# xuzhougeng/minimap2_rs

Hardware: AMD Instinct MI355X
Metric: aligned Gbases/sec (PAF out), 10k×10kb ONT reads vs hg38, 1/2/4/8 GPUs (higher is better)
Workload: dtype int32

## Files before the change

include/mm2g.h:

```cpp
#ifndef MM2G_H
#define MM2G_H
#include <stdint.h>

#ifdef __cplusplus
extern "C" {
#endif

#define MM2G_OK 0
#define MM2G_E_ARG -1
#define MM2G_E_IO -2
#define MM2G_E_HIP -3
#define MM2G_E_NOMEM -4
#define MM2G_E_STATE -5
#define MM2G_E_UNSUP -6

typedef struct mm2g_index mm2g_index;
typedef struct mm2g_ctx mm2g_ctx;

int mm2g_version(void);
const char* mm2g_last_error(void);
int mm2g_device_count(void);

int mm2g_index_build_fasta(const char* path, int w, int k, int b, int flag, int n_threads, mm2g_index** out);
int mm2g_index_build_seqs(uint32_t n_seq, const char* const* names, const uint8_t* const* seqs, const uint64_t* lens,
// ... 146 lines not shown
    MM2G_KNOB_SKETCH_VIEW = 27,
    MM2G_KNOB_PRUNE_RESCUE = 29,
    MM2G_KNOB_VIEW_READS = 30,
    MM2G_KNOB_SEG_SPARSE = 31,
    MM2G_KNOB_SPEC_BATCH = 32,
    MM2G_KNOB_DV_PAR = 33,
    MM2G_KNOB_SEED_FUSE = 36,
    MM2G_KNOB_SKETCH_X32 = 37,
    MM2G_KNOB_BIG_WND = 38,
    MM2G_KNOB_CANDS_LONGW = 39,
    MM2G_KNOB_SEED_FUSE_BIG = 40,
    MM2G_KNOB_READ_TINY = 41,
    MM2G_KNOB_BIG_TINY = 42,
    MM2G_KNOB_SPEC_EVAL = 43,
    MM2G_KNOB_SMALL_REG = 44,
    MM2G_KNOB_COUNT = 45
};
int mm2g_ctx_set_knob(mm2g_ctx* ctx, int knob, int64_t value);
int64_t mm2g_ctx_get_knob(const mm2g_ctx* ctx, int knob);
enum {
    MM2G_IKNOB_IXCHUNK = 1,
    MM2G_IKNOB_IXPROF = 2,
    MM2G_IKNOB_LOAD_THREADS = 3,
    MM2G_IKNOB_GPU_STRICT = 4,
    MM2G_IKNOB_FORCE_FALLBACK = 5,
    MM2G_IKNOB_IXSORTV = 6,
    MM2G_IKNOB_COUNT = 7
};
int mm2g_set_index_knob(int knob, int64_t value);

int mm2g_prof_enable(mm2g_ctx* ctx, int on);
// ... 10 lines not shown
```

minimap2_rs_amd/_lib.py:

```python
from __future__ import annotations

import ctypes as C
import os

HERE = os.path.dirname(os.path.abspath(__file__))
BUILD_DIR = os.path.join(HERE, "build")
LIB_PATH = os.environ.get("MM2G_LIB") or os.path.join(BUILD_DIR, "libmm2g.so")
CLI_PATH = os.path.join(BUILD_DIR, "mm2rs")

MM2G_R_MAPPED = 1
MM2G_R_RESCUED = 2
MM2G_R_DV_FOUND = 4
MM2G_R_PANIC = 8
MM2G_R_EMPTY = 16


class MapOpts(C.Structure):
    _fields_ = [("w", C.c_int32), ("k", C.c_int32), ("max_gap", C.c_int32), ("bw", C.c_int32), ("bw_long", C.c_int32),
                ("min_cnt", C.c_int32), ("min_chain_score", C.c_int32), ("mask_level", C.c_float),
                ("pri_ratio", C.c_float), ("best_n", C.c_int32)]


class ReadResult(C.Structure):
    _fields_ = [("flags", C.c_int32), ("n_anchors", C.c_int32), ("score", C.c_int32), ("cm", C.c_int32),
# ... 19 lines not shown

class ChainResult(C.Structure):
    _fields_ = [("flags", C.c_int32), ("n_anchors", C.c_int32), ("score", C.c_int32), ("cm", C.c_int32), ("qs", C.c_int32),
                ("qe", C.c_int32), ("ts", C.c_int32), ("te", C.c_int32), ("rid", C.c_int32), ("rev", C.c_int32)]


class ChainLine(C.Structure):
    _fields_ = [("qs", C.c_int32), ("qe", C.c_int32), ("ts", C.c_int32), ("te", C.c_int32), ("rid", C.c_int32),
                ("rev", C.c_int32), ("cm", C.c_int32), ("primary", C.c_int32), ("dv", C.c_float), ("s1", C.c_int32),
                ("s2", C.c_int32)]


KNOBS = {"sort_small": 1, "seg_small": 2, "seg_chunk": 3, "giant_min": 4, "giant_min0": 5, "giant_lcap": 6, "giant_gmax": 7,
         "giant_gblocks": 8, "filter": 9, "lazy": 10, "prune": 11, "giant": 12, "sketch_prof": 13, "sort_prof": 14,
         "lseg_prof": 15, "midhist_bins": 16, "sync_each": 17, "host_threads": 18, "ws_min": 19,
         "sort_lds_kb": 20, "stop_at": 21, "spec_rounds": 22, "med_pairs": 23, "med_pairs_rescue": 24, "ws_fail": 25, "sketch_view": 27, "prune_rescue": 29, "view_reads": 30, "seg_sparse": 31, "spec_batch": 32, "dv_par": 33, "seed_fuse": 36, "sketch_x32": 37, "big_wnd": 38, "cands_longw": 39, "seed_fuse_big": 40, "read_tiny": 41, "big_tiny": 42, "spec_eval": 43, "small_reg": 44}
INDEX_KNOBS = {"ixchunk": 1, "ixprof": 2, "load_threads": 3, "gpu_strict": 4, "force_fallback": 5, "ixsortv": 6}
INDEX_ORIGINS = {1: "host build", 2: "gpu build", 3: "gpu build fell back to the host build", 4: ".mmi load"}

_VP = C.c_void_p
_P64 = C.POINTER(C.c_uint64)
_PI32 = C.POINTER(C.c_int32)

SIGNATURES = {
    "mm2g_version": (C.c_int, []),
    "mm2g_last_error": (C.c_char_p, []),
    "mm2g_device_count": (C.c_int, []),
    "mm2g_index_build_fasta": (C.c_int, [C.c_char_p, C.c_int, C.c_int, C.c_int, C.c_int, C.c_int, C.POINTER(_VP)]),
    "mm2g_index_build_seqs": (C.c_int, [C.c_uint32, C.POINTER(C.c_char_p), C.POINTER(C.c_void_p), _P64,
                                        C.c_int, C.c_int, C.c_int, C.c_int, C.c_int, C.POINTER(_VP)]),
    "mm2g_index_build_fasta_gpu": (C.c_int, [C.c_char_p, C.c_int, C.c_int, C.c_int, C.c_int, C.c_int, C.c_int, C.POINTER(_VP)]),
# ... 78 lines not shown
```

minimap2_rs_amd/csrc/mm2g_host.hip:

```cpp
#include <hip/hip_runtime.h>

#include <algorithm>
#include <cmath>
#include <cstdarg>
#include <cstdio>
#include <cstring>
#include <map>
#include <memory>
#include <mutex>
#include <string>
#include <atomic>
#include <thread>
#include <vector>

#include "../../include/mm2g.h"
#include "mm2g_index.h"
#include "mm2g_internal.h"
#include "mm2g_multi.h"
#include "mm2g_reads.h"

using namespace mm2g;

static thread_local std::string g_err;
static int set_err(int code, const char* fmt, ...) {
// ... 78 lines not shown
    case MM2G_KNOB_SKETCH_VIEW: return 2560;
    case MM2G_KNOB_PRUNE_RESCUE: return 1;
    case MM2G_KNOB_VIEW_READS: return 2048;
    case MM2G_KNOB_SEG_SPARSE: return 1;
    case MM2G_KNOB_SPEC_BATCH: return 4;
    case MM2G_KNOB_DV_PAR: return 1;
    case MM2G_KNOB_SEED_FUSE: return 1;
    case MM2G_KNOB_SEED_FUSE_BIG: return 1;
    case MM2G_KNOB_READ_TINY: return 16;
    case MM2G_KNOB_BIG_TINY: return 16;
    case MM2G_KNOB_SPEC_EVAL: return 1;
    case MM2G_KNOB_SMALL_REG: return 1;
    case MM2G_KNOB_SKETCH_X32: return 1;
    case MM2G_KNOB_BIG_WND: return 126;
    case MM2G_KNOB_CANDS_LONGW: return 1024;
    case MM2G_KNOB_HOST_THREADS: return (int64_t)std::max(1u, std::min(8u, std::thread::hardware_concurrency()));
    default: return 0;
    }
}

struct mm2g_ctx {
    int device = 0;
    hipStream_t stream = nullptr;
    int64_t knob[MM2G_KNOB_COUNT] = {};
    const HostIndex* hidx = nullptr;
    struct DevIndex { DevBuf tab, ix_pos, goff; uint32_t cells = 0; };
    std::shared_ptr<DevIndex> dix;
    uint32_t log2cap = 0;
    int32_t mid_occ = 10;
    bool have_index = false;
// ... 953 lines not shown
}

static int enqueue_sort(mm2g_ctx* c, const mm2g_map_opts* o, MapBatch& B) {
    const uint32_t n = B.n;
    const int64_t* K = c->knob;
    SeedArgs sa = seed_args(c, o, B);
    sa.keys = B.keys; sa.cap_keys = c->keys.cap / 8;
    sa.order = B.rorder;
    sa.fuse_mmax = B.fuse_mmax; sa.small_max = B.sort_small_max; sa.fuse_big = B.fuse_big;
    {
        ProfScope ps(c, "seed_write");
        LCHK(launch_seed_write(sa, grid_for(n), c->stream));
    }
    uint32_t* rlist;
    ENSURE(c->cnt2, uint32_t, n, B.cnt2);
    ENSURE(c->rlist, uint32_t, n + 2, rlist);
    ENSURE(c->smax, uint64_t, n, B.smax);
    SortArgs so{};
    so.n = n; so.a_off = B.a_off; so.keys = B.keys; so.tmp = B.ktmp;
    so.qb = B.kl.qb; so.rb = B.kl.rb; so.n_seq = B.kl.n_seq;
    so.cap_keys = c->keys.cap / 8;
    so.goff = (const uint32_t*)c->dix->goff.p;
    so.cells = B.filt ? c->dix->cells : 0u;
    so.cnt2 = B.cnt2; so.smax = B.smax;
    so.small_max = B.sort_small_max;
    so.seg_small = (uint32_t)std::max<int64_t>(1, std::min<int64_t>(K[MM2G_KNOB_SEG_SMALL], SEG_THREAD));
    so.abort = B.st32;
    so.meta = (uint32_t*)c->fbuf.p;
    so.rlist = rlist; so.rcount = rlist + n; so.rwork = rlist + n + 1;
    so.order = B.rorder;
    so.lds_words = (uint32_t)(std::max<int64_t>(0, K[MM2G_KNOB_SORT_LDS_KB]) * 256);
    so.fuse_mmax = B.fuse_mmax;
    so.fuse_big = B.fuse_big; so.a_part = B.a_part;
    so.read_tiny = (uint32_t)std::max<int64_t>(1, std::min<int64_t>(K[MM2G_KNOB_READ_TINY], 1024));
    so.big_tiny = (uint32_t)std::max<int64_t>(1, std::min<int64_t>(K[MM2G_KNOB_BIG_TINY], 2048));
    so.small_reg = K[MM2G_KNOB_SMALL_REG] ? 1u : 0u;
    so.big_wnd = (uint32_t)std::max<int64_t>(0, K[MM2G_KNOB_BIG_WND]);
    so.rd_off = c->d_rd_off; so.mz_base = B.mz_base; so.mz_cnt = B.mz_cnt; so.mz_y = B.mz_y;
    so.mz_n = B.mz_n; so.mz_poff = B.mz_poff; so.ix_pos = (const uint64_t*)c->dix->ix_pos.p; so.kl = B.kl; so.span = o->k;
    so.cap_pos = c->dix->ix_pos.cap / 8;
    uint64_t* sprof = nullptr;
    if (K[MM2G_KNOB_SORT_PROF]) { HIPCHK(hipMalloc(&sprof, (size_t)n * 192)); HIPCHK(hipMemsetAsync(sprof, 0, (size_t)n * 192, c->stream)); so.prof = sprof; }
    if (K[MM2G_KNOB_STOP_AT] == 1) return 0;
    {
        ProfScope ps(c, "sort_small");
// ... 71 lines not shown
    }
    if (n == 0) {
        HIPCHK(hipMemcpyAsync(c->h_stat, B.st, STAT_WORDS * 8, hipMemcpyDeviceToHost, c->stream));
        HIPCHK(hipEventRecord(c->ev_done, c->stream));
        c->mapped = true;
        return 0;
    }
    if (int e = run_sketch(c, o->w, o->k, c->sk1, (int32_t*)B.st32, B.out, B.st)) return e;
    B.mcap = c->sk1.cap;
    B.mz_base = (const uint64_t*)c->sk1.base.p; B.mz_cnt = (const uint32_t*)c->sk1.cnt.p;
    B.mz_x = (const uint64_t*)c->sk1.x.p; B.mz_y = (const uint32_t*)c->sk1.y.p;
    if (int e = enqueue_filter(c, o, B)) return e;
    if (int e = enqueue_seed_count(c, o, B)) return e;
    B.filt = !full && !stop_after_sort && K[MM2G_KNOB_FILTER] && std::max(mdx0, mdx1) <= (1 << CELL_SHIFT);
    B.sort_small_max = (uint32_t)std::min<int64_t>(K[MM2G_KNOB_SORT_SMALL], 4096);
    if (B.filt && K[MM2G_KNOB_SEED_FUSE]) {
        SortArgs t{};
        t.cells = c->dix->cells;
        t.lds_words = (uint32_t)(std::max<int64_t>(0, K[MM2G_KNOB_SORT_LDS_KB]) * 256);
        const uint32_t LW = sort_read_lds_words(t), nw = (t.cells + 31) / 32;
        if (LW > 2 * nw + 64 + 2048) B.fuse_mmax = std::min<uint32_t>((LW - 2 * nw - 64 - 2048) / 4, 0xffffu);
    }
    B.fuse_big = (B.filt && K[MM2G_KNOB_SEED_FUSE_BIG]) ? 1u : 0u;
    c->filt_last = B.filt; c->small_last = B.sort_small_max;
    if (int e = enqueue_sort(c, o, B)) return e;
    const int64_t stop_at = K[MM2G_KNOB_STOP_AT];
    const bool chain = !stop_after_sort && stop_at != 1 && stop_at != 2;
    if (chain) {
        ChainJob J;
        J.n = n; J.rd_off = c->d_rd_off; J.a_off = B.a_off; J.a_cnt = B.a_cnt;
        J.keys = B.keys; J.ktmp = B.ktmp; J.cnt2 = B.cnt2; J.smax = B.smax;
        J.out = B.out; J.abort = B.st32; J.stat = B.st;
        J.P0.max_dist_x = mdx0; J.P0.max_dist_y = std::max(o->max_gap, o->bw); J.P0.bw = o->bw; J.P0.max_iter = 5000; J.P0.max_skip = 25;
        J.P0.span = o->k; J.P0.rescue_size = 1000; J.P0.rescue_ratio_f = 1.0f - 0.1f; J.P0.pass = 0; J.P0.lut_n = o->bw + 1;
        J.P0.multi = multi ? 1 : 0;
        J.gap = 0.01f * 0.8f * (float)o->k;
        J.npass = stop_at == 3 ? 1 : 2;
        J.mdx1 = mdx1; J.mdy1 = std::max(o->max_gap, o->bw_long); J.bw_long = o->bw_long;
// ... 713 lines not shown
```

minimap2_rs_amd/csrc/mm2g_internal.h:

```cpp
#pragma once
#include <stdint.h>

namespace mm2g {

constexpr uint64_t U64MAX = ~0ULL;
constexpr int WAVE = 64;
constexpr int CHAIN_TINY = 8;
constexpr int CHAIN_MED = 128;

struct KeyLayout {
    uint32_t qb, rb, gb;
    uint32_t n_seq;
};

struct ReadOut {
    int32_t flags;
    int32_t n_anchors;
    int32_t score;
    int32_t cm;
    int32_t qs, qe, ts, te;
    int32_t group;
    int32_t best_i;
    int32_t n_match;
    int32_t dv_st, dv_en;
// ... 122 lines not shown
    uint64_t cap_keys = 0;
    const uint32_t* goff = nullptr;
    uint32_t cells = 0;
    uint32_t* cnt2 = nullptr;
    uint64_t* smax = nullptr;
    uint32_t small_max = 0;
    uint64_t* prof = nullptr;
    uint32_t lds_words = 0;
    uint32_t seg_small = 0;
    uint32_t* meta = nullptr;
    const uint32_t* abort = nullptr;
    uint32_t* rlist = nullptr;
    uint32_t* rcount = nullptr;
    const uint32_t* order = nullptr;
    uint32_t* rwork = nullptr;
    uint32_t big_wnd = 1u << 30;
    uint32_t fuse_mmax = 0;
    const uint64_t* rd_off = nullptr; const uint64_t* mz_base = nullptr; const uint32_t* mz_cnt = nullptr;
    const uint32_t* mz_y = nullptr; const uint32_t* mz_n = nullptr; const uint32_t* mz_poff = nullptr;
    const uint64_t* ix_pos = nullptr; KeyLayout kl{}; int span = 0; uint64_t cap_pos = 0;
    uint32_t fuse_big = 0;
    const uint32_t* a_part = nullptr;
    uint32_t read_tiny = 16, big_tiny = 16;
    uint32_t small_reg = 1;
};
struct ChainArgs {
    uint32_t n = 0;
    const uint64_t* rd_off = nullptr;
    const uint64_t* a_off = nullptr;
    const uint64_t* keys = nullptr;
// ... 111 lines not shown
```

minimap2_rs_amd/csrc/mm2g_kernels.hip:

```cpp
#include <hip/hip_runtime.h>
#include <stdint.h>
#include <limits.h>
#include <algorithm>
#include <type_traits>
#include "mm2g_internal.h"

using namespace mm2g;

#define DEVI __device__ __forceinline__

#ifdef MM2G_CHECKED
__device__ unsigned long long g_chk[4];
DEVI uint64_t ck_idx(uint64_t i, uint64_t cap, int line) {
    if (i < cap) return i;
    if (atomicCAS(&g_chk[0], 0ULL, (unsigned long long)line) == 0ULL) { g_chk[1] = i; g_chk[2] = cap; }
    return 0;
}
#define CK(i, cap) ck_idx((uint64_t)(i), (uint64_t)(cap), __LINE__)
#define TRACE(tr, slot, v) do { if (tr) __hip_atomic_store(&(tr)[slot], (uint32_t)(v), __ATOMIC_RELAXED, __HIP_MEMORY_SCOPE_SYSTEM); } while (0)
#else
#define TRACE(tr, slot, v) do {} while (0)
#define CK(i, cap) (i)
#endif

// ... 7 lines not shown
DEVI void wave_lds_sync() {
    __builtin_amdgcn_fence(__ATOMIC_RELEASE, "wavefront");
    __builtin_amdgcn_wave_barrier();
    __builtin_amdgcn_fence(__ATOMIC_ACQUIRE, "wavefront");
}
DEVI void vm_drain() { asm volatile("s_waitcnt vmcnt(0)" ::: "memory"); }

DEVI int32_t rdl(int32_t v, int l) { return __builtin_amdgcn_readlane(v, l); }
DEVI uint32_t rdlu(uint32_t v, int l) { return (uint32_t)__builtin_amdgcn_readlane((int)v, l); }
DEVI uint64_t rdl64(uint64_t v, int l) {
    uint32_t lo = (uint32_t)__builtin_amdgcn_readlane((int)(uint32_t)v, l);
    uint32_t hi = (uint32_t)__builtin_amdgcn_readlane((int)(uint32_t)(v >> 32), l);
    return ((uint64_t)hi << 32) | lo;
}
DEVI int32_t uni(int32_t v) { return __builtin_amdgcn_readfirstlane(v); }

DEVI int32_t shr1(int32_t v, int32_t in0) {
    const int32_t t = __shfl_up(v, 1, 64);
    return lane_id() == 0 ? in0 : t;
}

template <typename T, typename F>
DEVI T wave_incl_scan(T v, F op) {
    const int l = lane_id();
#pragma unroll
    for (int d = 1; d < 64; d <<= 1) {
        T o = __shfl_up(v, d, 64);
        if (l >= d) v = op(o, v);
    }
    return v;
}
// ... 857 lines not shown
#pragma unroll
                for (int r = 0; r < KPT; ++r) {
                    const uint64_t y = s[(t ^ m) * KPT + r];
                    x[r] = (lowt == up) ? (x[r] < y ? x[r] : y) : (x[r] > y ? x[r] : y);
                }
            }
        }
    }
    __syncthreads();
#pragma unroll
    for (int r = 0; r < KPT; ++r) s[t * KPT + r] = x[r];
    __syncthreads();
}

__global__ __launch_bounds__(256) void k_sort_small(SortArgs a) {
    if (blockIdx.x == 0 && threadIdx.x == 0) { *a.rcount = 0; if (a.rwork) *a.rwork = 0; }
    if (a.abort && (*a.abort & BS_ANCHORS)) return;
    __shared__ uint64_t s[SORT_SMALL];
    const uint32_t r = blockIdx.x;
    if (r >= a.n) return;
    const uint64_t base = a.a_off[r];
    const uint32_t A = (uint32_t)(a.a_off[r + 1] - base);
    if (A > a.small_max) return;
    if (threadIdx.x == 0) { a.cnt2[r] = A; a.smax[r] = 0; }
    if (A == 1 && threadIdx.x == 0) a.tmp[CK(base, a.cap_keys)] = a.keys[CK(base, a.cap_keys)];
    if (A <= 1) return;
    uint32_t np = 1; while (np < A) np <<= 1;
    uint64_t* K = a.keys;
    for (uint32_t i = threadIdx.x; i < np; i += blockDim.x) s[i] = i < A ? K[CK(base + i, a.cap_keys)] : U64MAX;
    __syncthreads();
    if (np >= 512 && a.small_reg) {
// ... 328 lines not shown
#undef NS_STEP
}

DEVI void scan_lb(int32_t& a, int32_t& b) {
    constexpr int32_t NEG = -(1 << 29);
#define LB_STEP(CTRL, RM)                                                   \
    {                                                                       \
        const int32_t oa = dpp<CTRL, RM>(0, a), ob = dpp<CTRL, RM>(NEG, b); \
        b = max(ob + a, b); a = max(oa + a, NEG);                           \
    }
    LB_STEP(0x111, 0xf) LB_STEP(0x112, 0xf) LB_STEP(0x114, 0xf) LB_STEP(0x118, 0xf)
    LB_STEP(0x142, 0xa) LB_STEP(0x143, 0xc)
#undef LB_STEP
}

template <bool GL, int NT>
__global__ __launch_bounds__(NT) void k_sort_read(SortArgs a) {
    constexpr int NW = NT / 64;
    if (a.abort && (*a.abort & BS_ANCHORS)) return;
    __shared__ uint64_t red[32];
    __shared__ uint32_t s_sc[16], s_kept, s_nbig;
    __shared__ uint2 s_big[BIG_MAX];
    __shared__ uint32_t s_goff[GOFF_LDS];
    extern __shared__ uint64_t dyn64[];
    uint32_t* dyn = (uint32_t*)dyn64;
    if (blockIdx.x >= a.n) return;
    const uint32_t r = a.order ? a.order[blockIdx.x] : blockIdx.x;
    const uint64_t base = a.a_off[r];
    const uint32_t A0 = (uint32_t)(a.a_off[r + 1] - base);
    if (A0 <= a.small_max) return;
#ifdef MM2G_CHECKED
    if (base + A0 > a.cap_keys) { if (threadIdx.x == 0) CK(base + A0, a.cap_keys); return; }
#endif
    const int tid = threadIdx.x, lane = lane_id();
    uint64_t* const pq = a.prof ? a.prof + (uint64_t)r * 24 : nullptr;
    if (pq && tid == 0) pq[10] = pq[12] = wall_clock64();
#define SORT_PH(k) do { if (pq && tid == 0) { const uint64_t t_ = wall_clock64(); pq[k] += t_ - pq[12]; pq[12] = t_; } } while (0)
#define SORT_END(nb, nk) do { if (pq && tid == 0) { pq[8] = A0; pq[9] = ((uint64_t)(nb) << 32) | (nk); pq[11] = wall_clock64(); } } while (0)
    const uint32_t qb = a.qb, gsh = a.qb + a.rb;
    const uint64_t rmask = (1ULL << a.rb) - 1;
    uint64_t* K = a.keys + base;
    uint64_t* O = a.tmp + base;
    const bool filt = a.cells != 0;
    const uint32_t ng = 2u * a.n_seq + 2u;
    if (!GL && filt) {
        for (uint32_t i = tid; i < ng && i < (uint32_t)GOFF_LDS; i += NT) s_goff[i] = a.goff[i];
    }
    if (tid == 0) { s_nbig = 0; s_kept = 0; }
    __syncthreads();
    auto cell_of = [&](uint64_t x) -> uint32_t {
        const uint32_t g = (uint32_t)(x >> gsh);
        return (GL ? a.goff[g] : s_goff[g]) + 1u + (uint32_t)(((x >> qb) & rmask) >> CELL_SHIFT);
    };
    const uint32_t nw = (a.cells + 31) >> 5;
    const uint32_t LW = a.lds_words;
    uint32_t* B1 = dyn;
    uint32_t* B2 = dyn + nw;
    auto defer = [&]() { if (tid == 0) { a.rlist[atomicAdd(a.rcount, 1u)] = r; SORT_END(0xffffu, 0u); } };
    if (!filt || A0 > 65535u) { defer(); return; }
    {
        for (uint32_t i = tid; i < 2 * nw; i += NT) dyn[i] = 0;
        const uint32_t fm = a.fuse_mmax ? a.mz_cnt[r] : 0u;
        if (a.fuse_mmax && fm <= a.fuse_mmax) {
            uint32_t* Mi = dyn + 2 * nw;
            uint32_t* Mp = Mi + fm;
            uint32_t* My = Mp + fm;
            uint32_t* Mh = My + fm;
            const uint64_t mb = a.mz_base[r];
            if (tid == 0 && a.abort) {
                atomicAdd(stat_word(a.abort, ST_FUSED_ANCHORS), (unsigned long long)A0);
                atomicAdd(stat_word(a.abort, ST_FUSED_MZ), (unsigned long long)fm);
            }
            uint32_t carry = 0;
            constexpr int FS = 2;
            for (uint32_t i0 = 0; i0 < fm; i0 += NT * FS) {
                uint32_t nraw[FS], po[FS], yy[FS], cs = 0;
#pragma unroll
                for (int j = 0; j < FS; ++j) {
                    const uint32_t i = i0 + (uint32_t)tid * FS + (uint32_t)j;
                    const bool v = i < fm;
                    nraw[j] = v ? a.mz_n[mb + i] : 0u;
                    po[j] = v ? a.mz_poff[mb + i] : 0u; yy[j] = v ? a.mz_y[mb + i] : 0u;
                }
#pragma unroll
                for (int j = 0; j < FS; ++j) cs += ix_count(nraw[j]);
                uint32_t tot;
                uint32_t run = carry + block_excl_sum<NW>(cs, tot, s_sc);
#pragma unroll
                for (int j = 0; j < FS; ++j) {
                    const uint32_t i = i0 + (uint32_t)tid * FS + (uint32_t)j;
                    run += ix_count(nraw[j]);
                    if (i < fm) { Mi[i] = run; Mp[i] = po[j]; My[i] = yy[j]; Mh[i] = nraw[j]; }
                }
                carry += tot;
            }
            __syncthreads();
            uint16_t* O16 = (uint16_t*)(Mh + fm);
            const uint32_t nb16 = (A0 + 15) >> 4;
            for (uint32_t i = tid; i < fm; i += NT) {
                const uint32_t lo = i ? Mi[i - 1] : 0u, hi = Mi[i];
                for (uint32_t b = (lo + 15) >> 4; (b << 4) < hi; ++b) O16[b] = (uint16_t)i;
            }
            __syncthreads();
            SORT_PH(3);
            const int32_t qlen = (int32_t)(a.rd_off[r + 1] - a.rd_off[r]);
            constexpr int FU = SORT_FUSE_U;
            for (uint32_t i0 = 0; i0 < A0; i0 += NT * FU) {
                uint32_t lo[FU], hi[FU];
#pragma unroll
                for (int u = 0; u < FU; ++u) {
                    const uint32_t t = i0 + (uint32_t)u * NT + tid, b = t < A0 ? t >> 4 : 0u;
                    lo[u] = O16[b];
                    hi[u] = t >= A0 ? lo[u] : (b + 1 < nb16 ? (uint32_t)O16[b + 1] : fm - 1);
                }
                while (true) {
                    bool act = false;
#pragma unroll
                    for (int u = 0; u < FU; ++u) {
                        if (lo[u] < hi[u]) {
                            const uint32_t t = i0 + (uint32_t)u * NT + tid, mid = (lo[u] + hi[u]) >> 1;
// ... 63 lines not shown
            const uint32_t b1 = B1[w];
            const uint32_t nb = (b1 << 1) | (w ? B1[w - 1] >> 31 : 0u) | (b1 >> 1) | (w + 1 < nw ? B1[w + 1] << 31 : 0u);
            const uint32_t kc = b1 & (B2[w] | nb);
            B2[w] = kc;
            loc += (uint32_t)__popc(kc);
        }
        uint32_t nkc;
        uint32_t run = block_excl_sum<NW>(loc, nkc, s_sc);
        for (uint32_t w = wa; w < wb; ++w) { B1[w] = run; run += (uint32_t)__popc(B2[w]); }
        SORT_PH(0);
        if (pq && tid == 0) pq[13] = nkc;
        const uint32_t cw = (nkc + 1) >> 1;
        const uint32_t cofs = LW >= cw + 2 ? (LW - cw) & ~1u : 0u;
        const uint32_t kbits = gsh + (32u - (uint32_t)__builtin_clz(2u * a.n_seq | 1u));
        const uint32_t W = cofs >> 1;
        if (kbits > 48u || qb + CELL_SHIFT > 32u || cofs < 2 * nw || W < SEG_RANK) { defer(); return; }
        {
            constexpr uint64_t kmask = (1ULL << 48) - 1;
            uint32_t* C = dyn + cofs;
            uint64_t* S = dyn64;
            for (uint32_t i = tid; i < cw; i += NT) C[i] = 0;
            __syncthreads();
            auto c16 = [&](uint32_t rk) -> uint32_t { return (C[rk >> 1] >> ((rk & 1) << 4)) & 0xffffu; };
            uint64_t smx = 0;
            uint16_t* T16 = (uint16_t*)(a.meta + base);
            for (uint32_t i0 = 0; i0 < A0; i0 += NT * SORT_U2) {
                uint64_t x[SORT_U2];
                uint32_t c[SORT_U2], kw[SORT_U2], pw[SORT_U2];
#pragma unroll
                for (int u = 0; u < SORT_U2; ++u) { const uint32_t i = i0 + (uint32_t)u * NT + tid; x[u] = i < A0 ? K[i] : 0; }
#pragma unroll
                for (int u = 0; u < SORT_U2; ++u) c[u] = cell_of(x[u]);
#pragma unroll
                for (int u = 0; u < SORT_U2; ++u) { kw[u] = B2[c[u] >> 5]; pw[u] = B1[c[u] >> 5]; }
#pragma unroll
                for (int u = 0; u < SORT_U2; ++u) {
                    const uint32_t i = i0 + (uint32_t)u * NT + tid;
                    if (i < A0) {
                        const uint32_t b = c[u] & 31;
                        const bool kept = (kw[u] >> b) & 1u;
                        const uint32_t rk = pw[u] + (uint32_t)__popc(kw[u] & ((1u << b) - 1u));
                        if (kept) atomicAdd(&C[rk >> 1], 1u << ((rk & 1) << 4));
                        else smx = x[u] + 1 > smx ? x[u] + 1 : smx;
                        T16[i] = kept ? (uint16_t)rk : (uint16_t)0xffffu;
                    }
                }
            }
            smx = block_max64<NW>(smx, red);
            const uint32_t per2 = (cw + NT - 1) / NT;
            const uint32_t ca = min(cw, (uint32_t)tid * per2), cb = min(cw, ca + per2);
            uint32_t l2 = 0;
            for (uint32_t i = ca; i < cb; ++i) { const uint32_t v = C[i]; l2 += (v & 0xffffu) + (v >> 16); }
            uint32_t A;
            uint32_t o = block_excl_sum<NW>(l2, A, s_sc);
            for (uint32_t i = ca; i < cb; ++i) {
                const uint32_t v = C[i], lo = v & 0xffffu;
                C[i] = o | ((o + lo) << 16);
                o += lo + (v >> 16);
            }
            if (tid == 0) { a.cnt2[r] = A; a.smax[r] = smx; }
            __syncthreads();
            SORT_PH(1);
            auto offx = [&](uint32_t rk) -> uint32_t { return rk < nkc ? c16(rk) : A; };
            uint32_t ra = 0;
            while (ra < nkc) {
                const uint32_t oa = c16(ra);
                uint32_t lo = ra + 1, hi = nkc;
                while (lo < hi) { const uint32_t mid = (lo + hi + 1) >> 1; if (offx(mid) <= oa + W) lo = mid; else hi = mid - 1; }
                const uint32_t rb = lo;
                const uint32_t ob = offx(rb);
                if (ob > oa + W) {
                    __syncthreads();
                    if (tid == 0) s_kept = 0;
                    __syncthreads();
                    block_pass_kmu<8, NT>(K, T16, A0, [&](uint32_t, uint64_t x, uint16_t m, bool valid) {
                        const bool mine = valid && (uint32_t)m == ra;
                        const uint64_t mb = ballot(mine);
// ... 12 lines not shown
                    __syncthreads();
                    SORT_PH(2);
                    ra = ra + 1;
                    continue;
                }
                const uint32_t nwin = ob - oa;
                __syncthreads();
                block_pass_km<SORT_UG, NT>(K, T16, A0, [&](uint32_t, uint64_t x, uint16_t m) {
                    const uint32_t rk = m;
                    if (m != 0xffffu && rk >= ra && rk < rb) {
                        const uint32_t sh = (rk & 1) << 4;
                        const uint32_t pos = ((atomicAdd(&C[rk >> 1], 1u << sh) >> sh) & 0xffffu) - oa;
                        S[pos] = x | ((uint64_t)rk << 48);
                    }
                });
                __syncthreads();
                SORT_PH(2);
                if (pq && tid == 0) pq[7] += 1;
                auto seg_of = [&](uint64_t x, uint32_t& s, uint32_t& e) {
                    const uint32_t rk = (uint32_t)(x >> 48);
                    s = (rk ? c16(rk - 1) : 0u) - oa;
                    e = c16(rk) - oa;
                };
                const uint32_t nch = (nwin + 63) >> 6;
                for (uint32_t q = (uint32_t)wave_id(); q < nch; q += 2 * NW) {
                    const uint32_t ia = q * 64 + (uint32_t)lane, ib = ia + NW * 64;
                    const bool va = ia < nwin, vb = ib < nwin;
                    uint64_t xa = S[va ? ia : 0], xb = S[vb ? ib : 0];
                    uint32_t sa, ea, sb, eb;
                    seg_of(xa, sa, ea);
                    seg_of(xb, sb, eb);
                    xa = va ? xa : U64MAX; xb = vb ? xb : U64MAX;
                    const bool na = any(va && ea - sa > a.read_tiny && ea - sa <= a.seg_small);
                    const bool nb = any(vb && eb - sb > a.read_tiny && eb - sb <= a.seg_small);
                    if (na) { wave_bitonic64_np(xa); if (va) S[ia] = xa; }
                    if (nb) { wave_bitonic64_np(xb); if (vb) S[ib] = xb; }
                }
                __syncthreads();
                SORT_PH(4);
                const uint32_t* S32 = (const uint32_t*)S;
                uint32_t pc_tiny = 0, pc_long = 0, pc_srch = 0;
                for (uint32_t i = tid; i < nwin; i += NT) {
                    const uint64_t x = S[i];
                    uint32_t s, e;
                    seg_of(x, s, e);
                    const uint32_t L = e - s;
                    if (L > a.seg_small) {
                        O[oa + i] = x & kmask;
                        if (i == s) {
                            const uint32_t slot = atomicAdd(&s_nbig, 1u);
                            if (slot < (uint32_t)BIG_MAX) s_big[slot] = make_uint2(oa + s, oa + e);
                        }
                        continue;
                    }
// ... 11 lines not shown
                        for (uint32_t c = s >> 6; c <= (e - 1) >> 6; ++c) {
                            if (c == co) continue;
                            rank += count_below_lo(S32, max(s, c << 6), min(e, (c << 6) + 64), xl, c < co);
                        }
                    }
                    O[oa + s + rank] = x & kmask;
                }
                if (pq) {
                    const uint64_t v14 = wave_sum64(((uint64_t)pc_long << 32) | pc_tiny), v15 = wave_sum64(pc_srch);
                    if (lane == 0) { atomicAdd((unsigned long long*)&pq[14], (unsigned long long)v14); atomicAdd((unsigned long long*)&pq[15], (unsigned long long)v15); }
                }
                __syncthreads();
                SORT_PH(5);
                ra = rb;
            }
            const uint32_t nbig = s_nbig;
            bool big_radix = nbig > (uint32_t)BIG_MAX;
            for (uint32_t b = 0; b < nbig && !big_radix; ++b) big_radix = s_big[b].y - s_big[b].x > SEG_RANK;
            if (big_radix) { defer(); return; }
            {
                for (uint32_t b = 0; b < nbig; ++b) {
                    const uint2 sg = s_big[b];
                    const uint32_t L = sg.y - sg.x;
                    if (L <= SEG_RANK) {
                        __syncthreads();
                        block_pass8<4, NT>(O + sg.x, L, [&](uint32_t i, uint64_t x) { dyn64[i] = x; });
                        __syncthreads();
                        constexpr int KPT = (int)SEG_RANK / NT;
                        uint64_t xk[KPT];
                        uint32_t rk[KPT];
#pragma unroll
                        for (int u = 0; u < KPT; ++u) { const uint32_t iu = (uint32_t)tid + (uint32_t)u * NT; xk[u] = iu < L ? dyn64[iu] : U64MAX; rk[u] = 0; }
                        const int nu = (int)((L + NT - 1) / NT);
                        for (uint32_t j = 0; j < L; ++j) {
                            const uint64_t y = dyn64[j];
#pragma unroll
                            for (int u = 0; u < KPT; ++u) {
                                const uint32_t iu = (uint32_t)tid + (uint32_t)u * NT;
                                if (u < nu) rk[u] += (y < xk[u] || (y == xk[u] && j < iu)) ? 1u : 0u;
                            }
                        }
                        __syncthreads();
#pragma unroll
                        for (int u = 0; u < KPT; ++u) { const uint32_t iu = (uint32_t)tid + (uint32_t)u * NT; if (iu < L) O[sg.x + rk[u]] = xk[u]; }
                    }
                }
            }
            SORT_PH(6);
            SORT_END(nbig, A);
            return;
        }
    }
#undef SORT_PH
#undef SORT_END
}

template <bool GL>
__global__ __launch_bounds__(1024) void k_sort_radix(SortArgs a) {
    if (a.abort && (*a.abort & BS_ANCHORS)) return;
    __shared__ uint64_t red[32];
    __shared__ uint32_t s_kept;
    __shared__ uint32_t s_goff[GOFF_LDS];
    extern __shared__ uint64_t dyn64[];
    uint32_t* dyn = (uint32_t*)dyn64;
    const int tid = threadIdx.x, lane = lane_id();
    const uint32_t nlist = *a.rcount;
    const uint32_t qb = a.qb, gsh = a.qb + a.rb;
    const uint64_t rmask = (1ULL << a.rb) - 1;
    const bool filt = a.cells != 0;
// ... 2538 lines not shown
    return 0;
}
uint32_t sort_read_lds_words(const SortArgs& a) {
    const size_t bmb = (size_t)2 * ((a.cells + 31) / 32) * 4;
    size_t lds = std::max<size_t>(a.lds_words ? (size_t)a.lds_words * 4 : (size_t)SORT_LDS, bmb);
    return (uint32_t)(std::min<size_t>(lds, (size_t)SORT_LDS) / 4);
}
int launch_sort_read(SortStage stage, const SortArgs& a, hipStream_t st) {
    if (a.n == 0) return 0;
    if (stage == SortStage::Small) hipLaunchKernelGGL(k_sort_small, dim3(a.n), dim3(256), 0, st, a);
    else if (stage == SortStage::Read) {
        const size_t lds = (size_t)sort_read_lds_words(a) * 4;
        SortArgs b = a;
        b.lds_words = (uint32_t)(lds / 4);
        const bool gl = 2u * b.n_seq + 2u > (uint32_t)GOFF_LDS;
#define SR_LAUNCH(G, T) hipLaunchKernelGGL((k_sort_read<G, T>), dim3(a.n), dim3(T), lds, st, b)
        if (lds <= (size_t)SORT_LDS_HALF) {
            if (gl) SR_LAUNCH(true, 512);
            else SR_LAUNCH(false, 512);
        } else if (gl) SR_LAUNCH(true, 1024);
        else SR_LAUNCH(false, 1024);
#undef SR_LAUNCH
    } else if (stage != SortStage::Listed) {
        return (int)hipErrorInvalidValue;
    } else if (a.cells) {
        SortArgs b = a;
        b.lds_words = (uint32_t)(SORT_LDS / 4);
        const int ncu = cu_count(256);
        const unsigned grid = std::min<uint32_t>(a.n, (uint32_t)std::max(ncu, 1));
        if (2u * b.n_seq + 2u > (uint32_t)GOFF_LDS) hipLaunchKernelGGL(k_sort_big<true>, dim3(grid), dim3(1024), (size_t)SORT_LDS, st, b);
        else hipLaunchKernelGGL(k_sort_big<false>, dim3(grid), dim3(1024), (size_t)SORT_LDS, st, b);
// ... 148 lines not shown
```

Measured before the change: 19.32.

## Make per-read sort kernel persistent with atomic work-taking and next-read prefetch

Turns k_sort_read into a persistent kernel. A grid sized to CU slots pulls read indices from an atomic counter (rtake) instead of launching one block per read. While finishing the current read, it prefetches the next read's header (offsets, minimizer counts) and, when small enough, its first minimizer tile into registers, so the load latency overlaps with compute. The persistent mode is on by default through a new knob. It adds loop-carried state and double-buffered shared headers, which increases register pressure and the risk of synchronisation bugs. It also guards the fused seeding paths on the presence of cells.

```diff
diff --git a/include/mm2g.h b/include/mm2g.h
--- a/include/mm2g.h
+++ b/include/mm2g.h
@@ -184,7 +184,9 @@
     MM2G_KNOB_BIG_TINY = 42,
     MM2G_KNOB_SPEC_EVAL = 43,
     MM2G_KNOB_SMALL_REG = 44,
-    MM2G_KNOB_COUNT = 45
+    MM2G_KNOB_SORT_PERSIST = 45,
+    MM2G_KNOB_SORT_GRID = 46,
+    MM2G_KNOB_COUNT = 47
 };
 int mm2g_ctx_set_knob(mm2g_ctx* ctx, int knob, int64_t value);
 int64_t mm2g_ctx_get_knob(const mm2g_ctx* ctx, int knob);
diff --git a/minimap2_rs_amd/_lib.py b/minimap2_rs_amd/_lib.py
--- a/minimap2_rs_amd/_lib.py
+++ b/minimap2_rs_amd/_lib.py
@@ -57,7 +57,8 @@
 KNOBS = {"sort_small": 1, "seg_small": 2, "seg_chunk": 3, "giant_min": 4, "giant_min0": 5, "giant_lcap": 6, "giant_gmax": 7,
          "giant_gblocks": 8, "filter": 9, "lazy": 10, "prune": 11, "giant": 12, "sketch_prof": 13, "sort_prof": 14,
          "lseg_prof": 15, "midhist_bins": 16, "sync_each": 17, "host_threads": 18, "ws_min": 19,
-         "sort_lds_kb": 20, "stop_at": 21, "spec_rounds": 22, "med_pairs": 23, "med_pairs_rescue": 24, "ws_fail": 25, "sketch_view": 27, "prune_rescue": 29, "view_reads": 30, "seg_sparse": 31, "spec_batch": 32, "dv_par": 33, "seed_fuse": 36, "sketch_x32": 37, "big_wnd": 38, "cands_longw": 39, "seed_fuse_big": 40, "read_tiny": 41, "big_tiny": 42, "spec_eval": 43, "small_reg": 44}
+         "sort_lds_kb": 20, "stop_at": 21, "spec_rounds": 22, "med_pairs": 23, "med_pairs_rescue": 24, "ws_fail": 25, "sketch_view": 27, "prune_rescue": 29, "view_reads": 30, "seg_sparse": 31, "spec_batch": 32, "dv_par": 33, "seed_fuse": 36, "sketch_x32": 37, "big_wnd": 38, "cands_longw": 39, "seed_fuse_big": 40, "read_tiny": 41, "big_tiny": 42, "spec_eval": 43, "small_reg": 44,
+         "sort_persist": 45, "sort_grid": 46}
 INDEX_KNOBS = {"ixchunk": 1, "ixprof": 2, "load_threads": 3, "gpu_strict": 4, "force_fallback": 5, "ixsortv": 6}
 INDEX_ORIGINS = {1: "host build", 2: "gpu build", 3: "gpu build fell back to the host build", 4: ".mmi load"}
 
diff --git a/minimap2_rs_amd/csrc/mm2g_host.hip b/minimap2_rs_amd/csrc/mm2g_host.hip
--- a/minimap2_rs_amd/csrc/mm2g_host.hip
+++ b/minimap2_rs_amd/csrc/mm2g_host.hip
@@ -116,6 +116,7 @@
     case MM2G_KNOB_SKETCH_X32: return 1;
     case MM2G_KNOB_BIG_WND: return 126;
     case MM2G_KNOB_CANDS_LONGW: return 1024;
+    case MM2G_KNOB_SORT_PERSIST: return 1;
     case MM2G_KNOB_HOST_THREADS: return (int64_t)std::max(1u, std::min(8u, std::thread::hardware_concurrency()));
     default: return 0;
     }
@@ -1099,7 +1100,7 @@
     }
     uint32_t* rlist;
     ENSURE(c->cnt2, uint32_t, n, B.cnt2);
-    ENSURE(c->rlist, uint32_t, n + 2, rlist);
+    ENSURE(c->rlist, uint32_t, n + 3, rlist);
     ENSURE(c->smax, uint64_t, n, B.smax);
     SortArgs so{};
     so.n = n; so.a_off = B.a_off; so.keys = B.keys; so.tmp = B.ktmp;
@@ -1114,6 +1115,8 @@
     so.meta = (uint32_t*)c->fbuf.p;
     so.rlist = rlist; so.rcount = rlist + n; so.rwork = rlist + n + 1;
     so.order = B.rorder;
+    so.rtake = rlist + n + 2;
+    so.persist = !K[MM2G_KNOB_SORT_PERSIST] ? 0u : K[MM2G_KNOB_SORT_GRID] > 0 ? (uint32_t)std::min<int64_t>(K[MM2G_KNOB_SORT_GRID], 1 << 20) : 0xffffffffu;
     so.lds_words = (uint32_t)(std::max<int64_t>(0, K[MM2G_KNOB_SORT_LDS_KB]) * 256);
     so.fuse_mmax = B.fuse_mmax;
     so.fuse_big = B.fuse_big; so.a_part = B.a_part;
@@ -1215,14 +1218,15 @@
     if (int e = enqueue_seed_count(c, o, B)) return e;
     B.filt = !full && !stop_after_sort && K[MM2G_KNOB_FILTER] && std::max(mdx0, mdx1) <= (1 << CELL_SHIFT);
     B.sort_small_max = (uint32_t)std::min<int64_t>(K[MM2G_KNOB_SORT_SMALL], 4096);
-    if (B.filt && K[MM2G_KNOB_SEED_FUSE]) {
+    const bool have_cells = c->dix->cells != 0;
+    if (B.filt && have_cells && K[MM2G_KNOB_SEED_FUSE]) {
         SortArgs t{};
         t.cells = c->dix->cells;
         t.lds_words = (uint32_t)(std::max<int64_t>(0, K[MM2G_KNOB_SORT_LDS_KB]) * 256);
         const uint32_t LW = sort_read_lds_words(t), nw = (t.cells + 31) / 32;
         if (LW > 2 * nw + 64 + 2048) B.fuse_mmax = std::min<uint32_t>((LW - 2 * nw - 64 - 2048) / 4, 0xffffu);
     }
-    B.fuse_big = (B.filt && K[MM2G_KNOB_SEED_FUSE_BIG]) ? 1u : 0u;
+    B.fuse_big = (B.filt && have_cells && K[MM2G_KNOB_SEED_FUSE_BIG]) ? 1u : 0u;
     c->filt_last = B.filt; c->small_last = B.sort_small_max;
     if (int e = enqueue_sort(c, o, B)) return e;
     const int64_t stop_at = K[MM2G_KNOB_STOP_AT];
diff --git a/minimap2_rs_amd/csrc/mm2g_internal.h b/minimap2_rs_amd/csrc/mm2g_internal.h
--- a/minimap2_rs_amd/csrc/mm2g_internal.h
+++ b/minimap2_rs_amd/csrc/mm2g_internal.h
@@ -160,6 +160,8 @@
     uint32_t* rcount = nullptr;
     const uint32_t* order = nullptr;
     uint32_t* rwork = nullptr;
+    uint32_t persist = 0;
+    uint32_t* rtake = nullptr;
     uint32_t big_wnd = 1u << 30;
     uint32_t fuse_mmax = 0;
     const uint64_t* rd_off = nullptr; const uint64_t* mz_base = nullptr; const uint32_t* mz_cnt = nullptr;
diff --git a/minimap2_rs_amd/csrc/mm2g_kernels.hip b/minimap2_rs_amd/csrc/mm2g_kernels.hip
--- a/minimap2_rs_amd/csrc/mm2g_kernels.hip
+++ b/minimap2_rs_amd/csrc/mm2g_kernels.hip
@@ -45,7 +45,6 @@
     return ((uint64_t)hi << 32) | lo;
 }
 DEVI int32_t uni(int32_t v) { return __builtin_amdgcn_readfirstlane(v); }
-
 DEVI int32_t shr1(int32_t v, int32_t in0) {
     const int32_t t = __shfl_up(v, 1, 64);
     return lane_id() == 0 ? in0 : t;
@@ -933,7 +932,7 @@
 }
 
 __global__ __launch_bounds__(256) void k_sort_small(SortArgs a) {
-    if (blockIdx.x == 0 && threadIdx.x == 0) { *a.rcount = 0; if (a.rwork) *a.rwork = 0; }
+    if (blockIdx.x == 0 && threadIdx.x == 0) { *a.rcount = 0; if (a.rwork) *a.rwork = 0; if (a.rtake) *a.rtake = 0; }
     if (a.abort && (*a.abort & BS_ANCHORS)) return;
     __shared__ uint64_t s[SORT_SMALL];
     const uint32_t r = blockIdx.x;
@@ -1292,6 +1291,8 @@
 #undef LB_STEP
 }
 
+struct SortHdr { uint64_t base, mb; uint32_t r, A0, fm, qlen; };
+constexpr uint32_t SORT_NONE = 0xffffffffu;
 template <bool GL, int NT>
 __global__ __launch_bounds__(NT) void k_sort_read(SortArgs a) {
     constexpr int NW = NT / 64;
@@ -1300,32 +1301,18 @@
     __shared__ uint32_t s_sc[16], s_kept, s_nbig;
     __shared__ uint2 s_big[BIG_MAX];
     __shared__ uint32_t s_goff[GOFF_LDS];
+    __shared__ SortHdr s_hdr[2];
     extern __shared__ uint64_t dyn64[];
     uint32_t* dyn = (uint32_t*)dyn64;
-    if (blockIdx.x >= a.n) return;
-    const uint32_t r = a.order ? a.order[blockIdx.x] : blockIdx.x;
-    const uint64_t base = a.a_off[r];
-    const uint32_t A0 = (uint32_t)(a.a_off[r + 1] - base);
-    if (A0 <= a.small_max) return;
-#ifdef MM2G_CHECKED
-    if (base + A0 > a.cap_keys) { if (threadIdx.x == 0) CK(base + A0, a.cap_keys); return; }
-#endif
+    if (!a.rtake && blockIdx.x >= a.n) return;
     const int tid = threadIdx.x, lane = lane_id();
-    uint64_t* const pq = a.prof ? a.prof + (uint64_t)r * 24 : nullptr;
-    if (pq && tid == 0) pq[10] = pq[12] = wall_clock64();
-#define SORT_PH(k) do { if (pq && tid == 0) { const uint64_t t_ = wall_clock64(); pq[k] += t_ - pq[12]; pq[12] = t_; } } while (0)
-#define SORT_END(nb, nk) do { if (pq && tid == 0) { pq[8] = A0; pq[9] = ((uint64_t)(nb) << 32) | (nk); pq[11] = wall_clock64(); } } while (0)
     const uint32_t qb = a.qb, gsh = a.qb + a.rb;
     const uint64_t rmask = (1ULL << a.rb) - 1;
-    uint64_t* K = a.keys + base;
-    uint64_t* O = a.tmp + base;
     const bool filt = a.cells != 0;
     const uint32_t ng = 2u * a.n_seq + 2u;
     if (!GL && filt) {
         for (uint32_t i = tid; i < ng && i < (uint32_t)GOFF_LDS; i += NT) s_goff[i] = a.goff[i];
     }
-    if (tid == 0) { s_nbig = 0; s_kept = 0; }
-    __syncthreads();
     auto cell_of = [&](uint64_t x) -> uint32_t {
         const uint32_t g = (uint32_t)(x >> gsh);
         return (GL ? a.goff[g] : s_goff[g]) + 1u + (uint32_t)(((x >> qb) & rmask) >> CELL_SHIFT);
@@ -1334,31 +1321,73 @@
     const uint32_t LW = a.lds_words;
     uint32_t* B1 = dyn;
     uint32_t* B2 = dyn + nw;
+    auto load_hdr = [&](uint32_t b, SortHdr& h) {
+        h.r = SORT_NONE; h.A0 = 0; h.fm = 0; h.qlen = 0; h.base = 0; h.mb = 0;
+        if (b >= a.n) return;
+        const uint32_t rr = a.order ? a.order[b] : b;
+        h.r = rr;
+        h.base = a.a_off[rr];
+        h.A0 = (uint32_t)(a.a_off[rr + 1] - h.base);
+        if (a.fuse_mmax) { h.fm = a.mz_cnt[rr]; h.mb = a.mz_base[rr]; h.qlen = (uint32_t)(a.rd_off[rr + 1] - a.rd_off[rr]); }
+    };
+    constexpr int FS = 2;
+    uint32_t pf_n[FS], pf_p[FS], pf_y[FS];
+#pragma unroll
+    for (int j = 0; j < FS; ++j) pf_n[j] = pf_p[j] = pf_y[j] = 0;
+    uint32_t cur = 0;
+    bool pre = false, pf_on = false;
+#define SORT_NEXT(p) { if (!a.rtake) return; pre = (p); cur ^= (p) ? 1u : 0u; continue; }
+    for (;;) {
+    __syncthreads();
+    if (tid == 0) {
+        if (!pre) load_hdr(a.rtake ? atomicAdd(a.rtake, 1u) : blockIdx.x, s_hdr[cur]);
+        s_nbig = 0; s_kept = 0;
+    }
+    if (!pre) pf_on = false;
+    __syncthreads();
+    const uint32_t r = (uint32_t)uni((int32_t)s_hdr[cur].r);
+    if (r == SORT_NONE) return;
+    const uint64_t base = uni64(s_hdr[cur].base);
+    const uint32_t A0 = (uint32_t)uni((int32_t)s_hdr[cur].A0);
+    if (A0 <= a.small_max) SORT_NEXT(false);
+#ifdef MM2G_CHECKED
+    if (base + A0 > a.cap_keys) { if (threadIdx.x == 0) CK(base + A0, a.cap_keys); SORT_NEXT(false); }
+#endif
+    uint64_t* const pq = a.prof ? a.prof + (uint64_t)r * 24 : nullptr;
+    if (pq && tid == 0) pq[10] = pq[12] = wall_clock64();
+#define SORT_PH(k) do { if (pq && tid == 0) { const uint64_t t_ = wall_clock64(); pq[k] += t_ - pq[12]; pq[12] = t_; } } while (0)
+#define SORT_END(nb, nk) do { if (pq && tid == 0) { pq[8] = A0; pq[9] = ((uint64_t)(nb) << 32) | (nk); pq[11] = wall_clock64(); } } while (0)
+    uint64_t* K = a.keys + base;
+    uint64_t* O = a.tmp + base;
     auto defer = [&]() { if (tid == 0) { a.rlist[atomicAdd(a.rcount, 1u)] = r; SORT_END(0xffffu, 0u); } };
-    if (!filt || A0 > 65535u) { defer(); return; }
+    if (!filt || A0 > 65535u) { defer(); SORT_NEXT(false); }
     {
         for (uint32_t i = tid; i < 2 * nw; i += NT) dyn[i] = 0;
-        const uint32_t fm = a.fuse_mmax ? a.mz_cnt[r] : 0u;
+        const uint32_t fm = (uint32_t)uni((int32_t)s_hdr[cur].fm);
         if (a.fuse_mmax && fm <= a.fuse_mmax) {
             uint32_t* Mi = dyn + 2 * nw;
             uint32_t* Mp = Mi + fm;
             uint32_t* My = Mp + fm;
             uint32_t* Mh = My + fm;
-            const uint64_t mb = a.mz_base[r];
+            const uint64_t mb = uni64(s_hdr[cur].mb);
             if (tid == 0 && a.abort) {
                 atomicAdd(stat_word(a.abort, ST_FUSED_ANCHORS), (unsigned long long)A0);
                 atomicAdd(stat_word(a.abort, ST_FUSED_MZ), (unsigned long long)fm);
             }
             uint32_t carry = 0;
-            constexpr int FS = 2;
             for (uint32_t i0 = 0; i0 < fm; i0 += NT * FS) {
                 uint32_t nraw[FS], po[FS], yy[FS], cs = 0;
-#pragma unroll
-                for (int j = 0; j < FS; ++j) {
-                    const uint32_t i = i0 + (uint32_t)tid * FS + (uint32_t)j;
-                    const bool v = i < fm;
-                    nraw[j] = v ? a.mz_n[mb + i] : 0u;
-                    po[j] = v ? a.mz_poff[mb + i] : 0u; yy[j] = v ? a.mz_y[mb + i] : 0u;
+                if (pf_on) {
+#pragma unroll
+                    for (int j = 0; j < FS; ++j) { nraw[j] = pf_n[j]; po[j] = pf_p[j]; yy[j] = pf_y[j]; }
+                } else {
+#pragma unroll
+                    for (int j = 0; j < FS; ++j) {
+                        const uint32_t i = i0 + (uint32_t)tid * FS + (uint32_t)j;
+                        const bool v = i < fm;
+                        nraw[j] = v ? a.mz_n[mb + i] : 0u;
+                        po[j] = v ? a.mz_poff[mb + i] : 0u; yy[j] = v ? a.mz_y[mb + i] : 0u;
+                    }
                 }
 #pragma unroll
                 for (int j = 0; j < FS; ++j) cs += ix_count(nraw[j]);
@@ -1381,7 +1410,7 @@
             }
             __syncthreads();
             SORT_PH(3);
-            const int32_t qlen = (int32_t)(a.rd_off[r + 1] - a.rd_off[r]);
+            const int32_t qlen = uni((int32_t)s_hdr[cur].qlen);
             constexpr int FU = SORT_FUSE_U;
             for (uint32_t i0 = 0; i0 < A0; i0 += NT * FU) {
                 uint32_t lo[FU], hi[FU];
@@ -1475,12 +1504,14 @@
         const uint32_t cofs = LW >= cw + 2 ? (LW - cw) & ~1u : 0u;
         const uint32_t kbits = gsh + (32u - (uint32_t)__builtin_clz(2u * a.n_seq | 1u));
         const uint32_t W = cofs >> 1;
-        if (kbits > 48u || qb + CELL_SHIFT > 32u || cofs < 2 * nw || W < SEG_RANK) { defer(); return; }
+        if (kbits > 48u || qb + CELL_SHIFT > 32u || cofs < 2 * nw || W < SEG_RANK) { defer(); SORT_NEXT(false); }
         {
             constexpr uint64_t kmask = (1ULL << 48) - 1;
             uint32_t* C = dyn + cofs;
             uint64_t* S = dyn64;
             for (uint32_t i = tid; i < cw; i += NT) C[i] = 0;
+            uint32_t nx_b = SORT_NONE, nx_r = SORT_NONE;
+            if (a.rtake && tid == 0) nx_b = atomicAdd(a.rtake, 1u);
             __syncthreads();
             auto c16 = [&](uint32_t rk) -> uint32_t { return (C[rk >> 1] >> ((rk & 1) << 4)) & 0xffffu; };
             uint64_t smx = 0;
@@ -1488,6 +1519,7 @@
             for (uint32_t i0 = 0; i0 < A0; i0 += NT * SORT_U2) {
                 uint64_t x[SORT_U2];
                 uint32_t c[SORT_U2], kw[SORT_U2], pw[SORT_U2];
+                if (i0 + NT * SORT_U2 >= A0 && a.rtake && tid == 0 && nx_b < a.n) nx_r = a.order ? a.order[nx_b] : nx_b;
 #pragma unroll
                 for (int u = 0; u < SORT_U2; ++u) { const uint32_t i = i0 + (uint32_t)u * NT + tid; x[u] = i < A0 ? K[i] : 0; }
 #pragma unroll
@@ -1508,6 +1540,12 @@
                 }
             }
             smx = block_max64<NW>(smx, red);
+            uint64_t nx_base = 0, nx_end = 0, nx_mb = 0, nx_q0 = 0, nx_q1 = 0;
+            uint32_t nx_fm = 0;
+            if (a.rtake && tid == 0 && nx_r != SORT_NONE) {
+                nx_base = a.a_off[nx_r]; nx_end = a.a_off[nx_r + 1];
+                if (a.fuse_mmax) { nx_fm = a.mz_cnt[nx_r]; nx_mb = a.mz_base[nx_r]; nx_q0 = a.rd_off[nx_r]; nx_q1 = a.rd_off[nx_r + 1]; }
+            }
             const uint32_t per2 = (cw + NT - 1) / NT;
             const uint32_t ca = min(cw, (uint32_t)tid * per2), cb = min(cw, ca + per2);
             uint32_t l2 = 0;
@@ -1522,6 +1560,12 @@
             if (tid == 0) { a.cnt2[r] = A; a.smax[r] = smx; }
             __syncthreads();
             SORT_PH(1);
+            auto put_hdr = [&]() {
+                SortHdr& h = s_hdr[cur ^ 1u];
+                h.r = nx_r; h.base = nx_base; h.A0 = (uint32_t)(nx_end - nx_base);
+                h.fm = nx_fm; h.mb = nx_mb; h.qlen = (uint32_t)(nx_q1 - nx_q0);
+            };
+            pf_on = false;
             auto offx = [&](uint32_t rk) -> uint32_t { return rk < nkc ? c16(rk) : A; };
             uint32_t ra = 0;
             while (ra < nkc) {
@@ -1564,6 +1608,7 @@
                         S[pos] = x | ((uint64_t)rk << 48);
                     }
                 });
+                if (a.rtake && tid == 0) put_hdr();
                 __syncthreads();
                 SORT_PH(2);
                 if (pq && tid == 0) pq[7] += 1;
@@ -1588,6 +1633,21 @@
                 }
                 __syncthreads();
                 SORT_PH(4);
+                if (a.rtake && rb >= nkc) {
+                    const uint32_t nr = (uint32_t)uni((int32_t)s_hdr[cur ^ 1u].r), nA = (uint32_t)uni((int32_t)s_hdr[cur ^ 1u].A0);
+                    const uint32_t nfm = (uint32_t)uni((int32_t)s_hdr[cur ^ 1u].fm);
+                    pf_on = nr != SORT_NONE && a.fuse_mmax && nfm <= a.fuse_mmax && nfm <= (uint32_t)(NT * FS) && nA > a.small_max && nA <= 65535u;
+                    if (pf_on) {
+                        const uint64_t nmb = uni64(s_hdr[cur ^ 1u].mb);
+#pragma unroll
+                        for (int j = 0; j < FS; ++j) {
+                            const uint32_t i = (uint32_t)tid * FS + (uint32_t)j;
+                            const bool v = i < nfm;
+                            pf_n[j] = v ? a.mz_n[nmb + i] : 0u;
+                            pf_p[j] = v ? a.mz_poff[nmb + i] : 0u; pf_y[j] = v ? a.mz_y[nmb + i] : 0u;
+                        }
+                    }
+                }
                 const uint32_t* S32 = (const uint32_t*)S;
                 uint32_t pc_tiny = 0, pc_long = 0, pc_srch = 0;
                 for (uint32_t i = tid; i < nwin; i += NT) {
@@ -1629,10 +1689,11 @@
                 SORT_PH(5);
                 ra = rb;
             }
+            if (a.rtake && tid == 0) put_hdr();
             const uint32_t nbig = s_nbig;
             bool big_radix = nbig > (uint32_t)BIG_MAX;
             for (uint32_t b = 0; b < nbig && !big_radix; ++b) big_radix = s_big[b].y - s_big[b].x > SEG_RANK;
-            if (big_radix) { defer(); return; }
+            if (big_radix) { defer(); SORT_NEXT(true); }
             {
                 for (uint32_t b = 0; b < nbig; ++b) {
                     const uint2 sg = s_big[b];
@@ -1663,11 +1724,13 @@
             }
             SORT_PH(6);
             SORT_END(nbig, A);
-            return;
-        }
+            SORT_NEXT(true);
+        }
+    }
     }
 #undef SORT_PH
 #undef SORT_END
+#undef SORT_NEXT
 }
 
 template <bool GL>
@@ -4236,7 +4299,12 @@
         SortArgs b = a;
         b.lds_words = (uint32_t)(lds / 4);
         const bool gl = 2u * b.n_seq + 2u > (uint32_t)GOFF_LDS;
-#define SR_LAUNCH(G, T) hipLaunchKernelGGL((k_sort_read<G, T>), dim3(a.n), dim3(T), lds, st, b)
+        uint32_t grid = a.n;
+        if (b.persist && b.rtake) {
+            const uint32_t slots = (uint32_t)std::max(cu_count(256), 1) * (lds <= (size_t)SORT_LDS_HALF ? 2u : 1u);
+            grid = std::min(a.n, std::min(slots, b.persist));
+        } else b.rtake = nullptr;
+#define SR_LAUNCH(G, T) hipLaunchKernelGGL((k_sort_read<G, T>), dim3(grid), dim3(T), lds, st, b)
         if (lds <= (size_t)SORT_LDS_HALF) {
             if (gl) SR_LAUNCH(true, 512);
             else SR_LAUNCH(false, 512);
```

Result: no change. 19.13 (-1.0%).
